# SxJyJay/MSMDFusion

Hardware: AMD Instinct MI355X
Metric: samples/sec MSMDFusion fwd+bwd nuScenes 0.075m voxel (MSMDFusion-LC sparse fusion path) (higher is better)
Workload: dtype f32 via 3xbf16 split MFMA (each fp32 operand = exact sum of 3 bf16 planes, 6 products, fp32 accumulate; fp32 storage); 1 GPU; configs[2]: MSMDFusion-LC sparse path (LiDAR SparseEncoder frozen + 4-scale virtual-point voxels + modality split + GMA-Conv + sparse_add + downscale -> BEV 640ch), fwd+bwd+AdamW, 2 x (28.7k LiDAR + 50k virtual pts)/GPU, 0.075 m voxels, fp32; global_batch=2, parallelism=dp1, index_prefetch=True, trainable_params=5654368

## Files before the change

### include/msmd_hip.h

```cpp
#ifndef MSMD_HIP_H_
#define MSMD_HIP_H_

#include <stddef.h>
#include <stdint.h>

#ifdef __cplusplus
extern "C" {
#endif

typedef void* msmd_stream_t;

enum msmd_status {
  MSMD_OK = 0,
  MSMD_ERR_INVALID_ARG = -1,
  MSMD_ERR_WORKSPACE = -2,
  MSMD_ERR_UNSUPPORTED = -3,
  MSMD_ERR_LAUNCH = -4,
  MSMD_ERR_RANGE = -5
};

const char* msmd_status_string(int status);
const char* msmd_last_launch_error(void);
int msmd_abi_version(void);
int msmd_device_ok(void);
// ... 122 lines not shown
  int32_t spatial_shape[3], ksize[3];
  int32_t method, reserved;
  int32_t* nbr;
} msmd_subm_desc;
size_t msmd_rulebook_subm3d_many_workspace_bytes(const msmd_subm_desc* descs, int n_desc);
int msmd_rulebook_subm3d_many(const msmd_subm_desc* descs, int n_desc, void* workspace,
                              size_t workspace_bytes, msmd_stream_t stream);

size_t msmd_rulebook_conv_workspace_bytes(int batch_size,
                                          const int* out_shape );

int msmd_rulebook_conv3d_count(const int32_t* indices , int n,
                               int batch_size, const int* out_shape,
                               const int* ksize, const int* stride,
                               const int* padding, int32_t* n_out ,
                               void* workspace, size_t workspace_bytes,
                               msmd_stream_t stream);

int msmd_rulebook_conv3d_fill(const int32_t* indices, int n, int batch_size,
                              const int* out_shape, const int* ksize,
                              const int* stride, const int* padding, int n_out,
                              int32_t* out_indices ,
                              int32_t* nbr_fwd ,
                              int32_t* nbr_bwd ,
                              void* workspace, size_t workspace_bytes,
                              msmd_stream_t stream);

int msmd_rulebook_deconv3d_count(const int32_t* indices , int n,
                                 int batch_size, const int* out_shape,
                                 const int* ksize, const int* stride,
                                 const int* padding, int32_t* n_out ,
                                 void* workspace, size_t workspace_bytes,
                                 msmd_stream_t stream);

int msmd_rulebook_deconv3d_fill(const int32_t* indices, int n, int batch_size,
                                const int* out_shape, const int* ksize,
                                const int* stride, const int* padding, int n_out,
                                int32_t* out_indices ,
                                int32_t* nbr_fwd ,
                                int32_t* nbr_bwd ,
                                void* workspace, size_t workspace_bytes,
                                msmd_stream_t stream);

size_t msmd_rulebook_conv_chain_workspace_bytes(int batch_size, int levels,
                                                const int* out_shapes);
int msmd_rulebook_conv3d_count_chain(const int32_t* indices, int n, int batch_size,
                                     int levels, const int* out_shapes, const int* ksizes,
                                     const int* strides, const int* paddings,
                                     int32_t* n_out , void* workspace,
                                     size_t workspace_bytes, msmd_stream_t stream);

size_t msmd_rulebook_add_conv_chain_workspace_bytes(int batch_size, int levels,
                                                    const int* in_shapes, const int* out_shapes);
int msmd_rulebook_add_conv_count_chain(const int32_t* const* extra, const int* n_extra,
                                       int batch_size, int levels, const int* in_shapes,
                                       const int* out_shapes, const int* ksizes,
                                       const int* strides, const int* paddings, int32_t* counts,
                                       void* workspace, size_t workspace_bytes,
                                       msmd_stream_t stream);

size_t msmd_rulebook_pairs_workspace_bytes(int kernel_volume, int n_rows);

int msmd_rulebook_pairs(const int32_t* nbr , int kernel_volume,
                        int n_rows, int32_t* indice_pairs ,
                        int ld, int32_t* indice_num , void* workspace,
                        size_t workspace_bytes, msmd_stream_t stream);

size_t msmd_spconv_packed_weight_elems(int kernel_volume, int c_in, int c_out);

int msmd_spconv_pack_weight(const float* weight, int kernel_volume, int c_in,
                            int c_out,
                            int flags ,
                            float* packed, msmd_stream_t stream);

int msmd_spconv_fwd_f32(const float* in_feat , int n_in,
                        int c_in, const float* packed_weight,
                        const int32_t* nbr , int ld, int n_out,
                        int kernel_volume, int weight_flip,
                        const int32_t* row_order ,
                        int32_t* tile_counter ,
                        float* out_feat , int c_out,
                        msmd_stream_t stream);

int msmd_spconv_fwd_split_supported(int c_in, int c_out, int kernel_volume);

size_t msmd_spconv_packed_split_bytes(int kernel_volume, int c_in ,
                                      int c_out , int planes);

int msmd_spconv_pack_weight_split(const float* weight, int kernel_volume, int c_in,
                                  int c_out, int flags ,
                                  int planes, void* packed, msmd_stream_t stream);
int msmd_spconv_pack_weight_split_pair(const float* weight, int kernel_volume, int c_in,
                                       int c_out, int flags, int planes, void* packed,
                                       void* packed_transposed, msmd_stream_t stream);

int msmd_spconv_pack_weight_split_many(const void* descs, int n_desc, long total_units,
                                       int planes, msmd_stream_t stream);

size_t msmd_spconv_fwd_split_workspace_bytes(int n_out, int c_out);

int msmd_spconv_fwd_split(const float* in_feat , int n_in, int c_in,
                          const void* packed_weight, const int32_t* nbr ,
                          int ld, int n_out, int kernel_volume, int weight_flip,
                          const int32_t* row_order ,
                          int32_t* tile_counter , int sync_ints,
                          float* out_feat , int c_out, int planes,
                          void* workspace, size_t workspace_bytes,
                          const int32_t* tile_prefix ,
                          msmd_stream_t stream);

int msmd_spconv_fwd_split_stats(const float* in_feat, int n_in, int c_in,
                                const void* packed_weight, const int32_t* nbr, int ld,
                                int n_out, int kernel_volume, int weight_flip,
                                const int32_t* row_order, int32_t* tile_counter, int sync_ints,
                                float* out_feat, int c_out, int planes, void* workspace,
                                size_t workspace_bytes, const int32_t* tile_prefix,
                                float* bn_partials, msmd_stream_t stream);
int msmd_spconv_fwd_split_stats_blocks(int n_out, int c_out);

int msmd_spconv_fwd_split_tile_rows(int c_out);

int msmd_spconv_fwd_split_instantiation(int c_out, int* params);

int msmd_rulebook_tile_prefix(const int32_t* nbr , int kernel_volume, int ld,
                              int n_rows, int rows_per_tile,
                              int32_t* prefix , msmd_stream_t stream);

int msmd_spconv_wgrad_split_supported(int c_in, int c_out);

int msmd_spconv_wgrad_split(const float* in_feat, int c_in, const float* d_out, int c_out,
                            const int32_t* indice_pairs ,
                            const int32_t* indice_num , int ld,
                            int kernel_volume, int planes,
                            float* d_weight ,
                            int krsc_out ,
                            void* workspace, size_t workspace_bytes, msmd_stream_t stream);

size_t msmd_rulebook_pair_segments_ints(int kernel_volume, int n_chunks);
int msmd_rulebook_pair_segments(const int32_t* indice_pairs ,
                                const int32_t* indice_num , int ld,
                                int kernel_volume, int chunk_rows, int n_chunks ,
                                int32_t* table ,
                                msmd_stream_t stream);
size_t msmd_spconv_wgrad_segments_workspace_bytes(int kernel_volume, int ld, int c_in, int c_out,
                                                  int n_chunks);
int msmd_spconv_wgrad_split_segments(const float* in_feat, int c_in, const float* d_out,
                                     int c_out, const int32_t* indice_pairs,
                                     const int32_t* indice_num, int ld, int kernel_volume,
                                     int planes, float* d_weight, int krsc_out,
                                     const int32_t* seg_table, int n_chunks, void* workspace,
                                     size_t workspace_bytes, msmd_stream_t stream);

int msmd_rulebook_permute_cols(const int32_t* nbr, int kernel_volume, int ld, int n,
                               const int32_t* order, int32_t* out ,
                               msmd_stream_t stream);

size_t msmd_rulebook_tiling_workspace_bytes(int n_rows, int rows_per_tile);
int msmd_rulebook_tiling(const int32_t* nbr, int kernel_volume, int n_rows,
                         int rows_per_tile, int32_t* order ,
                         int32_t* tiled , void* workspace,
                         size_t workspace_bytes, msmd_stream_t stream);

size_t msmd_rulebook_plan_workspace_bytes(int kernel_volume, int n_rows, int rows_per_tile);
int msmd_rulebook_plan(const int32_t* nbr, int kernel_volume, int n_rows,
                       int rows_per_tile, int32_t* order, int32_t* tiled,
                       int32_t* prefix128, int32_t* prefix256, int32_t* indice_pairs,
// ... 363 lines not shown
```

### msmdfusion_amd/_lib.py

```python
import ctypes as C
import os

import torch

_HERE = os.path.dirname(os.path.abspath(__file__))
LIB_PATH = os.environ.get("MSMD_LIB") or os.path.join(_HERE, "libmsmd_hip.so")

if not os.path.exists(LIB_PATH):
    raise RuntimeError(
        f"{LIB_PATH} is missing: the HIP library is not built. Run "
        "`make -C msmdfusion_amd/csrc` (hipcc, --offload-arch=gfx950). "
        "msmdfusion_amd has no fallback path.")

lib = (C.PyDLL if os.environ.get("MSMD_PYDLL") == "1" else C.CDLL)(LIB_PATH)

_vp, _i, _f, _sz = C.c_void_p, C.c_int, C.c_float, C.c_size_t
_i64 = C.c_int64
_ip = C.POINTER(C.c_int)
_fp = C.POINTER(C.c_float)

SIGNATURES = {
    "msmd_status_string": (C.c_char_p, [_i]),
    "msmd_last_launch_error": (C.c_char_p, []),
    "msmd_abi_version": (_i, []),
    "msmd_device_ok": (_i, []),
    "msmd_voxelize_workspace_bytes": (_sz, [_i, _i, _i]),
    "msmd_hard_voxelize": (_i, [_vp, _i, _i, _fp, _fp, _i, _i, _vp, _vp, _vp, _vp, _vp, _vp, _sz, _vp]),
    "msmd_hard_voxelize_many_workspace_bytes": (_sz, [_vp, _i]),
    "msmd_hard_voxelize_many": (_i, [_vp, _i, _vp, _sz, _vp]),
    "msmd_voxel_mean": (_i, [_vp, _vp, _i, _i, _i, _i, _vp, _vp]),
    "msmd_dynamic_voxelize": (_i, [_vp, _i, _i, _fp, _fp, _i, _vp, _vp]),
    "msmd_scatter_index_workspace_bytes": (_sz, [_i]),
    "msmd_scatter_index": (_i, [_vp, _i, _i, _vp, _vp, _vp, _vp, _vp, _vp, _vp, _sz, _vp]),
    "msmd_scatter_reduce_f32": (_i, [_vp, _i, _i, _vp, _vp, _i, _i, _vp, _vp, _vp]),
    "msmd_scatter_reduce_bwd_f32": (_i, [_vp, _i, _i, _i, _vp, _vp, _vp, _i, _vp, _vp]),
    "msmd_scatter_max_argmax_f32": (_i, [_vp, _i, _i, _vp, _vp, _i, _vp, _vp]),
    "msmd_scatter_gather_f32": (_i, [_vp, _i, _i, _vp, _i, _vp, _vp]),
    "msmd_roiaware_num_tiles": (_sz, [_i, _i]),
    "msmd_roiaware_count_workspace_bytes": (_sz, [_i, _i]),
    "msmd_roiaware_count": (_i, [_vp, _vp, _i, _vp, _vp, _i, _vp, _vp, _sz, _vp]),
    "msmd_roiaware_index_workspace_bytes": (_sz, [_i]),
    "msmd_roiaware_index": (_i, [_vp, _vp, _i, _vp, _vp, _i, _i, _i, _i, _i, _vp, _i, _vp, _vp, _vp,
                                 _vp, _vp, _sz, _vp]),
    "msmd_roiaware_pool_f32": (_i, [_vp, _i, _i, _vp, _vp, _i64, _i, _i, _i, _vp, _vp, _vp]),
    "msmd_roiaware_pool_bwd_f32": (_i, [_vp, _i64, _i, _vp, _i, _vp, _vp, _i, _vp, _i, _i, _vp, _vp]),
    "msmd_roiaware_write_table": (_i, [_vp, _vp, _i64, _i, _vp, _vp]),
    "msmd_roiaware_table_workspace_bytes": (_sz, [_i64, _i]),
    "msmd_roiaware_table_count": (_i, [_vp, _i64, _i, _vp, _vp, _sz, _vp]),
    "msmd_roiaware_table_index": (_i, [_vp, _i64, _i, _i, _i, _vp, _vp, _vp, _vp, _vp, _sz, _vp]),
    "msmd_points_in_boxes_f32": (_i, [_vp, _vp, _i, _i, _i, _i, _vp, _vp]),
    "msmd_rulebook_subm_workspace_bytes": (_sz, [_i]),
    "msmd_rulebook_subm3d": (_i, [_vp, _i, _i, _ip, _ip, _vp, _vp, _sz, _vp]),
    "msmd_rulebook_subm_bitmap_workspace_bytes": (_sz, [_i, _i, _ip]),
    "msmd_rulebook_subm3d_bitmap": (_i, [_vp, _i, _i, _ip, _ip, _vp, _vp, _sz, _vp]),
    "msmd_rulebook_conv_workspace_bytes": (_sz, [_i, _ip]),
    "msmd_rulebook_conv_chain_workspace_bytes": (_sz, [_i, _i, _ip]),
    "msmd_rulebook_conv3d_count_chain": (_i, [_vp, _i, _i, _i, _ip, _ip, _ip, _ip, _vp, _vp, _sz, _vp]),
    "msmd_rulebook_add_conv_chain_workspace_bytes": (_sz, [_i, _i, _ip, _ip]),
    "msmd_rulebook_add_conv_count_chain": (_i, [_vp, _ip, _i, _i, _ip, _ip, _ip, _ip, _ip, _vp, _vp,
                                                _sz, _vp]),
    "msmd_rulebook_conv3d_count": (_i, [_vp, _i, _i, _ip, _ip, _ip, _ip, _vp, _vp, _sz, _vp]),
    "msmd_rulebook_conv3d_fill": (_i, [_vp, _i, _i, _ip, _ip, _ip, _ip, _i, _vp, _vp, _vp, _vp, _sz, _vp]),
    "msmd_rulebook_deconv3d_count": (_i, [_vp, _i, _i, _ip, _ip, _ip, _ip, _vp, _vp, _sz, _vp]),
    "msmd_rulebook_deconv3d_fill": (_i, [_vp, _i, _i, _ip, _ip, _ip, _ip, _i, _vp, _vp, _vp, _vp, _sz,
                                         _vp]),
    "msmd_sparse_maxpool_fwd_f32": (_i, [_vp, _i, _i, _vp, _i, _i, _vp, _vp]),
    "msmd_sparse_maxpool_bwd_f32": (_i, [_vp, _vp, _vp, _i, _i, _vp, _i, _i, _vp, _vp]),
    "msmd_rulebook_pairs_workspace_bytes": (_sz, [_i, _i]),
    "msmd_rulebook_pairs": (_i, [_vp, _i, _i, _vp, _i, _vp, _vp, _sz, _vp]),
    "msmd_spconv_packed_weight_elems": (_sz, [_i, _i, _i]),
    "msmd_spconv_pack_weight": (_i, [_vp, _i, _i, _i, _i, _vp, _vp]),
    "msmd_spconv_fwd_f32": (_i, [_vp, _i, _i, _vp, _vp, _i, _i, _i, _i, _vp, _vp, _vp, _i, _vp]),
    "msmd_rulebook_row_masks": (_i, [_vp, _i, _i, _vp, _vp, _vp]),
    "msmd_rulebook_tile_costs": (_i, [_vp, _i, _i, _vp, _i, _vp, _vp]),
    "msmd_rulebook_tiling_workspace_bytes": (_sz, [_i, _i]),
    "msmd_rulebook_tiling": (_i, [_vp, _i, _i, _i, _vp, _vp, _vp, _sz, _vp]),
    "msmd_rulebook_plan_workspace_bytes": (_sz, [_i, _i, _i]),
    "msmd_rulebook_plan": (_i, [_vp, _i, _i, _i, _vp, _vp, _vp, _vp, _vp, _i, _vp, _vp, _sz, _vp]),
    "msmd_rulebook_subm3d_many_workspace_bytes": (_sz, [_vp, _i]),
    "msmd_rulebook_subm3d_many": (_i, [_vp, _i, _vp, _sz, _vp]),
    "msmd_rulebook_plan_many_workspace_bytes": (_sz, [_vp, _i]),
    "msmd_rulebook_plan_many": (_i, [_vp, _i, _vp, _sz, _vp]),
    "msmd_spconv_wgrad_workspace_bytes": (_sz, [_i, _i, _i, _i]),
    "msmd_spconv_wgrad_f32": (_i, [_vp, _i, _vp, _i, _vp, _vp, _i, _i, _vp, _i, _vp, _sz, _vp]),
    "msmd_spconv_packed_split_bytes": (_sz, [_i, _i, _i, _i]),
    "msmd_spconv_pack_weight_split": (_i, [_vp, _i, _i, _i, _i, _i, _vp, _vp]),
    "msmd_spconv_pack_weight_split_pair": (_i, [_vp, _i, _i, _i, _i, _i, _vp, _vp, _vp]),
    "msmd_spconv_fwd_split_supported": (_i, [_i, _i, _i]),
    "msmd_spconv_fwd_split_workspace_bytes": (_sz, [_i, _i]),
    "msmd_spconv_fwd_split": (_i, [_vp, _i, _i, _vp, _vp, _i, _i, _i, _i, _vp, _vp, _i, _vp, _i, _i,
                                   _vp, _sz, _vp, _vp]),
    "msmd_spconv_fwd_split_stats": (_i, [_vp, _i, _i, _vp, _vp, _i, _i, _i, _i, _vp, _vp, _i, _vp, _i, _i, _vp, _sz, _vp, _vp, _vp]),
    "msmd_rulebook_tile_prefix": (_i, [_vp, _i, _i, _i, _i, _vp, _vp]),
    "msmd_spconv_fwd_split_tile_rows": (_i, [_i]),
    "msmd_spconv_fwd_split_instantiation": (_i, [_i, _ip]),
    "msmd_spconv_fwd_split_stats_blocks": (_i, [_i, _i]),
    "msmd_spconv_wgrad_split_supported": (_i, [_i, _i]),
    "msmd_spconv_wgrad_split": (_i, [_vp, _i, _vp, _i, _vp, _vp, _i, _i, _i, _vp, _i, _vp, _sz, _vp]),
    "msmd_spconv_pack_weight_split_many": (_i, [_vp, _i, C.c_long, _i, _vp]),
    "msmd_rulebook_pair_segments_ints": (_sz, [_i, _i]),
    "msmd_rulebook_pair_segments": (_i, [_vp, _vp, _i, _i, _i, _i, _vp, _vp]),
    "msmd_spconv_wgrad_segments_workspace_bytes": (_sz, [_i, _i, _i, _i, _i]),
    "msmd_spconv_wgrad_split_segments": (_i, [_vp, _i, _vp, _i, _vp, _vp, _i, _i, _i, _vp, _i, _vp,
                                              _i, _vp, _sz, _vp]),
    "msmd_rulebook_permute_cols": (_i, [_vp, _i, _i, _i, _vp, _vp, _vp]),
    "msmd_bn_workspace_bytes": (_sz, [_i, _i]),
    "msmd_bn_act_fwd_f32": (_i, [_vp, _vp, _i, _i, _vp, _vp, _vp, _vp, _i, _f, _f, _i, _vp, _vp, _vp, _vp, _sz, _vp]),
    "msmd_bn_act_fwd_from_partials_f32": (_i, [_vp, _vp, _i, _i, _vp, _vp, _vp, _vp, _f, _f, _i, _vp,
                                               _vp, _vp, _vp, _i, _vp]),
    "msmd_bn_act_bwd_f32": (_i, [_vp, _vp, _vp, _i, _i, _vp, _vp, _vp, _i, _i, _vp, _vp, _vp, _vp, _vp, _sz, _vp]),
    "msmd_bn_relu_bwd_f32": (_i, [_vp, _vp, _i, _i, _vp, _vp, _vp, _vp, _i, _vp, _vp, _vp, _vp, _sz, _vp]),
    "msmd_dense_scatter_f32": (_i, [_vp, _vp, _i, _i, _i, _ip, _vp, _vp]),
    "msmd_dense_gather_f32": (_i, [_vp, _vp, _i, _i, _i, _ip, _vp, _vp]),
    "msmd_bev_scatter_nhwc_f32": (_i, [_vp, _vp, _i, _i, _i, _ip, _vp, _i, _i, _vp]),
    "msmd_bev_gather_nhwc_f32": (_i, [_vp, _vp, _i, _i, _i, _ip, _vp, _i, _i, _vp]),
    "msmd_fg_gather_f32": (_i, [_vp, _vp, _i, _i, _i, _i, _vp, _i, _vp, C.c_double, _vp, _i, _vp, _i,
                                _vp, _vp, _vp, _vp, _vp]),
    "msmd_fg_gather_scored_f32": (_i, [_vp, _vp, _i, _i, _i, _i, _vp, _i, _vp, C.c_double, _vp, _i, _vp,
                                       _vp, _vp, _i, _i, _vp, _vp, _vp]),
    "msmd_fg_scatter_add_f32": (_i, [_vp, _i, _i, _vp, _i, _i, _i, _i, _i, _vp, _vp, _vp]),
    "msmd_depth_canvas_workspace_bytes": (_sz, [_i, _i, _i]),
    "msmd_boxes_overlap_bev_f32": (_i, [_vp, _i, _vp, _i, _vp, _vp]),
    "msmd_boxes_iou3d_f32": (_i, [_vp, _i, _vp, _i, _vp, _i, _i, _i, _i, _vp, _vp]),
    "msmd_heatmap_gaussian_f32": (_i, [_vp, _vp, _vp, _vp, _i, _i, _i, _i, _vp, _vp]),
    "msmd_gaussian_focal_workspace_bytes": (_sz, [_i64]),
    "msmd_gaussian_focal_f32": (_i, [_vp, _vp, _i64, _f, _vp, _vp, _vp, _sz, _vp]),
    "msmd_boxes_iou_bev_f32": (_i, [_vp, _i, _vp, _i, _vp, _vp]),
    "msmd_nms_workspace_bytes": (_sz, [_i, _i]),
    "msmd_nms_batched_f32": (_i, [_i, _vp, _i, _vp, _i, _i, _i, _vp, _i, _vp, _vp, _i, _vp, _vp, _sz,
                                  _vp]),
    "msmd_depth_canvas_f32": (_i, [_vp, _i, _vp, _i, _i, _i, _i, _vp, _vp, _vp, _sz, _vp]),
    "msmd_sparse_add_workspace_bytes": (_sz, [_i, _ip]),
    "msmd_sparse_add_count": (_i, [_vp, _i, _vp, _i, _i, _ip, _vp, _vp, _sz, _vp]),
    "msmd_sparse_add_fill": (_i, [_vp, _vp, _i, _vp, _vp, _i, _i, _i, _ip, _i, _vp, _vp, _vp, _vp, _vp, _sz, _vp]),
    "msmd_sparse_add_rows": (_i, [_vp, _vp, _i, _vp, _vp, _i, _i, _i, _vp, _vp]),
    "msmd_rows_inverse": (_i, [_vp, _i, _i, _vp, _vp]),
    "msmd_sparse_add_rows_gather": (_i, [_vp, _vp, _vp, _i, _vp, _vp, _vp, _i, _i, _i, _vp, _vp]),
    "msmd_gma_assemble_fwd_f32": (_i, [_vp, _i, _i, _vp, _i, _i, _vp, _vp, _vp, _i, _i, _vp, _vp, _vp, _vp,
                                       _i, _i, _vp, _vp]),
    "msmd_gma_assemble_bwd_f32": (_i, [_vp, _i, _i, _i, _i, _vp, _vp, _vp, _i, _i, _vp, _i, _i, _vp, _vp,
                                       _vp, _vp, _vp, _vp, _vp]),
    "msmd_gma_assemble_bwd_workspace_floats": (_sz, [_i]),
    "msmd_rows_linear_supported": (_i, [_i, _i]),
    "msmd_rows_linear_fwd_f32": (_i, [_vp, _i, _vp, _i, _i, _vp, _vp, _i, _i, _vp, _vp]),
    "msmd_rows_linear_bwd_workspace_bytes": (_sz, [_i, _i, _i]),
    "msmd_rows_linear_bwd_f32": (_i, [_vp, _i, _vp, _i, _i, _vp, _vp, _i, _i, _vp, _vp, _vp, _sz,
                                      _vp]),
    "msmd_modality_split_workspace_bytes": (_sz, [_i, _ip]),
    "msmd_modality_split": (_i, [_vp, _i, _vp, _i, _i, _ip, _vp, _vp, _vp, _vp, _vp, _vp, _sz, _vp]),
    "msmd_modality_split_stats": (_i, [_vp, _i, _vp, _i, _i, _ip, _vp, _vp, _vp, _vp, _vp, _vp, _vp, _sz,
                                       _vp]),
    "msmd_modality_split_float_keys_workspace_bytes": (_sz, [_i, _i, _i]),
    "msmd_modality_split_float_keys": (_i, [_vp, _i, _vp, _i, _i, _ip, _vp, _vp, _vp, _vp, _vp, _vp, _i,
                                            _vp, _sz, _vp]),
    "msmd_rows_where_workspace_bytes": (_sz, [_i]),
# ... 64 lines not shown
```

### msmdfusion_amd/kernels.py

```python
import ctypes as C
import os

import torch

from ._lib import check, float_arr, int3, lib


def _raw_stream(device_index=None):
    if device_index is None:
        device_index = torch._C._cuda_getDevice()
    return torch._C._cuda_getCurrentRawStream(device_index)


def _stream():
    return C.c_void_p(_raw_stream())


def _p(t):
    return None if t is None else t.data_ptr()


def _need_cuda(*ts):
    cur = None
    for t in ts:
# ... 953 lines not shown
        if want_seg and (WGRAD_CHUNK_ROWS > 0 or ld <= 0):
            want_seg = False
        o = dict(kvol=kvol, n=n, ld=ld, order=take(n), tiled=take(kvol * n) if want_table else None,
                 prefix={r: take((n + r - 1) // r + 1) for r in sorted(rows)},
                 pairs=take(kvol * 2 * ld) if want_pairs else None,
                 num=take(kvol) if want_pairs else None,
                 seg=take(int(lib.msmd_rulebook_pair_segments_ints(kvol, 1))) if want_seg else None)
        lay.append(o)
        d.nbr, d.kvol, d.n_rows, d.ld = t.data_ptr(), kvol, n, ld
    slab = torch.empty((max(total, 1),), dtype=torch.int32, device=dev)
    base = slab.data_ptr()
    at = lambda off: None if off is None else base + 4 * off
    for d, o in zip(descs, lay):
        d.order, d.tiled = at(o["order"]), at(o["tiled"])
        d.prefix128, d.prefix256 = at(o["prefix"].get(128)), at(o["prefix"].get(256))
        d.indice_pairs, d.indice_num, d.segtab = at(o["pairs"]), at(o["num"]), at(o["seg"])
    nbytes = lib.msmd_rulebook_plan_many_workspace_bytes(descs, len(jobs))
    ws = _ws(nbytes, dev)
    check(lib.msmd_rulebook_plan_many(descs, len(jobs), _p(ws), nbytes, _stream()),
          "msmd_rulebook_plan_many")
    def view(off, *shape):
        size = 1
        for v in shape:
            size *= v
        return slab[off:off + size].view(*shape)
    out = []
    for o in lay:
        kvol, n, ld = o["kvol"], o["n"], o["ld"]
        pairs = None
        if o["pairs"] is not None:
            pairs = (view(o["pairs"], kvol, 2, ld), view(o["num"], kvol))
        seg = None
        if o["seg"] is not None:
            seg = (slab[o["seg"]:o["seg"] + 3 * kvol + 1], 1)
        out.append(dict(order=view(o["order"], n),
                        tiled=None if o["tiled"] is None else view(o["tiled"], kvol, n),
                        prefix={r: slab[off:off + (n + r - 1) // r + 1]
                                for r, off in o["prefix"].items()},
                        pairs=pairs, segments=seg))
    return out


_TILE_COUNTERS = {}


_SYNC_INTS = 1 + 8192


def _tile_counter(device):
    key = (device, _raw_stream(device.index))
    c = _TILE_COUNTERS.get(key)
    if c is None:
        c = _TILE_COUNTERS[key] = torch.zeros((_SYNC_INTS,), dtype=torch.int32, device=device)
    return c


_EXCHANGE = {}


def _exchange_buffer(device, nbytes):
    key = (device, _raw_stream(device.index))
    b = _EXCHANGE.get(key)
    if b is None or b.numel() < nbytes:
        b = _EXCHANGE[key] = torch.empty((max(int(nbytes), 256),), dtype=torch.uint8,
                                         device=device)
    return b


def conv_forward(feat, packed_weight, nbr, n_out, c_out, weight_flip=False, row_order=None):
    _need_cuda(feat, packed_weight, nbr)
    f = feat.contiguous().float()
    n_in, c_in = f.shape
    kvol, ld = nbr.shape
    out = torch.empty((n_out, c_out), dtype=torch.float32, device=f.device)
    counter = _tile_counter(f.device) if row_order is not None else None
    _launch("spconv_fwd", lambda: check(
        lib.msmd_spconv_fwd_f32(_p(f), n_in, c_in, _p(packed_weight), _p(nbr), ld, int(n_out),
                                kvol, int(bool(weight_flip)), _p(row_order), _p(counter),
                                _p(out), int(c_out), _stream()), "msmd_spconv_fwd_f32"),
            nbr=nbr, c_in=c_in, c_out=int(c_out), n_in=n_in, n_out=int(n_out))
    return out


_SPLIT_SUPPORTED = {}


def split_supported(c_in, c_out, kvol=27):
    key = (c_in, c_out, kvol)
    v = _SPLIT_SUPPORTED.get(key)
    if v is None:
        v = _SPLIT_SUPPORTED[key] = bool(
            lib.msmd_spconv_fwd_split_supported(int(c_in), int(c_out), int(kvol)))
    return v


def pack_weight_split(weight, planes=3, transpose=False, krsc=False):
    _need_cuda(weight)
    w = weight.contiguous().float()
    if krsc:
        cout, cin = w.shape[0], w.shape[-1]
        kvol = w.numel() // (cout * cin)
    else:
        kvol, cin, cout = w.shape
    ci, co = (cout, cin) if transpose else (cin, cout)
    packed = torch.empty((lib.msmd_spconv_packed_split_bytes(kvol, ci, co, planes),),
                         dtype=torch.uint8, device=w.device)
    check(lib.msmd_spconv_pack_weight_split(_p(w), kvol, cin, cout,
                                            int(bool(transpose)) | (2 if krsc else 0), planes,
                                            _p(packed), _stream()),
          "msmd_spconv_pack_weight_split")
    return packed


def pack_weight_split_pair(weight, planes=3, krsc=False):
    _need_cuda(weight)
    w = weight.contiguous().float()
    if krsc:
        cout, cin = w.shape[0], w.shape[-1]
        kvol = w.numel() // (cout * cin)
    else:
        kvol, cin, cout = w.shape
    a = torch.empty((lib.msmd_spconv_packed_split_bytes(kvol, cin, cout, planes),),
                    dtype=torch.uint8, device=w.device)
    b = torch.empty((lib.msmd_spconv_packed_split_bytes(kvol, cout, cin, planes),),
                    dtype=torch.uint8, device=w.device)
    check(lib.msmd_spconv_pack_weight_split_pair(_p(w), kvol, cin, cout, 2 if krsc else 0, planes,
                                                 _p(a), _p(b), _stream()),
          "msmd_spconv_pack_weight_split_pair")
    return a, b


class _PackDesc(C.Structure):
    _fields_ = [("w", C.c_void_p), ("packed_a", C.c_void_p), ("packed_b", C.c_void_p),
                ("start", C.c_int64), ("kvol", C.c_int32), ("cin", C.c_int32),
                ("cout", C.c_int32), ("flags", C.c_int32)]


def pack_weight_split_many(jobs, planes=3):
    if not jobs:
        return
    descs = (_PackDesc * len(jobs))()
    start = 0
    keep = []
    for i, (weight, krsc, packed, packed_t) in enumerate(jobs):
        _need_cuda(weight, packed, packed_t)
        w = weight.detach()
        if not (w.is_contiguous() and w.dtype == torch.float32):
            w = w.contiguous().float()
        keep.append(w)
        if krsc:
            cout, cin = w.shape[0], w.shape[-1]
            kvol = w.numel() // (cout * cin)
        else:
            kvol, cin, cout = w.shape
        d = descs[i]
        d.w, d.packed_a = w.data_ptr(), packed.data_ptr()
        d.packed_b = packed_t.data_ptr() if packed_t is not None else None
        d.start, d.kvol, d.cin, d.cout, d.flags = start, kvol, cin, cout, 2 if krsc else 0
        start += lib.msmd_spconv_packed_split_bytes(kvol, cin, cout, planes) // (16 * planes)
        if packed_t is not None:
            start += lib.msmd_spconv_packed_split_bytes(kvol, cout, cin, planes) // (16 * planes)
    dev = jobs[0][0].device
    host = torch.frombuffer(bytearray(bytes(descs)), dtype=torch.uint8).pin_memory()
    table = host.to(dev, non_blocking=True)
    check(lib.msmd_spconv_pack_weight_split_many(_p(table), len(jobs), start, int(planes),
                                                 _stream()), "msmd_spconv_pack_weight_split_many")
# ... 1212 lines not shown
```

### msmdfusion_amd/spconv/functional.py

```python
import os
from collections import namedtuple

import torch
from torch.autograd import Function

from .. import kernels as K


def conv_planes():
    return int(os.environ.get("MSMD_CONV_PLANES", "3"))


SPLIT_MAX_FEATURE_BYTES = 0xFFFFFF00


def _use_split(c_in, c_out, kvol, n_in=0, planes=None):
    return ((conv_planes() if planes is None else planes) in (1, 2, 3)
            and n_in * c_in * 4 < SPLIT_MAX_FEATURE_BYTES and K.split_supported(c_in, c_out, kvol))


ConvNeeds = namedtuple("ConvNeeds", "fwd bwd wgrad_split want_pairs want_segments planes")


def conv_needs(c_in, c_out, kvol, n_in, n_out, need_grad, is_subm):
    planes = conv_planes()

    def ask(side, ci, co, n):
        if _use_split(ci, co, kvol, n, planes):
            return side, "split", K.split_tile_rows(co)
        return side, "ordered" if co >= 64 and ci % 16 == 0 else "plain", None
    bwd = ask("fwd" if is_subm else "bwd", c_out, c_in, n_out) if need_grad else None
    wgs = bool(need_grad) and K.wgrad_split_supported(c_in, c_out)
    return ConvNeeds(ask("fwd", c_in, c_out, n_in), bwd, wgs and planes in (1, 2, 3),
                     bool(need_grad), wgs, planes)


_F32_TILE_COUNTS = (12, 8, 6, 5, 4, 3, 2, 1)


def _conv_f32(x, weight, krsc, transpose, nbr, n_out, weight_flip=False, row_order=None):
    if krsc:
        c_out = weight.shape[-1] if transpose else weight.shape[0]
    else:
        c_out = weight.shape[1] if transpose else weight.shape[2]
    tiles = (c_out + 15) // 16
    if tiles in _F32_TILE_COUNTS:
        return K.conv_forward(x, _pack_f32(weight, transpose, krsc), nbr,
                              n_out, c_out, weight_flip=weight_flip, row_order=row_order)
    outs, c0 = [], 0
    while c0 < c_out:
        left = (c_out - c0 + 15) // 16
        width = min(16 * next(t for t in _F32_TILE_COUNTS if t <= left), c_out - c0)
        if krsc:
            w = weight[..., c0:c0 + width] if transpose else weight[c0:c0 + width]
        else:
            w = weight[:, c0:c0 + width, :] if transpose else weight[:, :, c0:c0 + width]
        outs.append(K.conv_forward(x, K.pack_weight(w, transpose=transpose, krsc=krsc), nbr,
                                   n_out, width, weight_flip=weight_flip, row_order=row_order))
        c0 += width
    return torch.cat(outs, 1)


_PACKS = {}
_F32_PACKS = {}


def _pack_entry(weight, np_, krsc, want_t):
    import weakref
    wid = id(weight)
    key = (weight.data_ptr(), tuple(weight.shape), np_, krsc, weight.device)
    e = _PACKS.get(wid)
    if e is None or e["ref"]() is not weight or e["key"] != key:
        if krsc:
            cout, cin = weight.shape[0], weight.shape[-1]
            kvol = weight.numel() // (cout * cin)
        else:
            kvol, cin, cout = weight.shape
        e = dict(ref=weakref.ref(weight, lambda _r, wid=wid: _PACKS.pop(wid, None)), key=key,
                 dims=(kvol, cin, cout), version=None, packed_t=None,
                 packed=torch.empty((K.lib.msmd_spconv_packed_split_bytes(kvol, cin, cout, np_),),
                                    dtype=torch.uint8, device=weight.device))
        _PACKS[wid] = e
    if want_t and e["packed_t"] is None:
        kvol, cin, cout = e["dims"]
        e["packed_t"] = torch.empty((K.lib.msmd_spconv_packed_split_bytes(kvol, cout, cin, np_),),
                                    dtype=torch.uint8, device=weight.device)
        e["version"] = None
    return e


def _packed_parameter(weight, np_, krsc, want_t):
    e = _pack_entry(weight, np_, krsc, want_t)
    if e["version"] != weight._version:
        jobs, entries = [], []
        for o in list(_PACKS.values()):
            w = o["ref"]()
            if w is None or o["key"][2] != np_ or o["key"][4] != weight.device:
                continue
            if o["version"] != w._version:
                jobs.append((w, o["key"][3], o["packed"], o["packed_t"]))
                entries.append((o, w._version))
        K.pack_weight_split_many(jobs, np_)
        for o, v in entries:
            o["version"] = v
    return e["packed"], e["packed_t"]


def _pack_f32(weight, transpose, krsc):
    if not isinstance(weight, torch.nn.Parameter):
        return K.pack_weight(weight, transpose=transpose, krsc=krsc)
    import weakref
    ck = (id(weight), bool(transpose))
    key = (weight.data_ptr(), weight._version, krsc, tuple(weight.shape))
    hit = _F32_PACKS.get(ck)
    if hit is not None and hit[0]() is weight and hit[1] == key:
        return hit[2]
    packed = K.pack_weight(weight, transpose=transpose, krsc=krsc)
    _F32_PACKS[ck] = (weakref.ref(weight, lambda _r, ck=ck: _F32_PACKS.pop(ck, None)), key, packed)
    return packed


def invalidate_packed_weights(weight=None):
    if weight is None:
        for e in _PACKS.values():
            e["version"] = None
        _F32_PACKS.clear()
        return
    e = _PACKS.get(id(weight))
    if e is not None:
        e["version"] = None
    for t in (False, True):
        _F32_PACKS.pop((id(weight), t), None)


def _conv_forward(features, weight, rb, krsc, want_dgrad, bn_stats=False):
    c_in, c_out = (weight.shape[-1], weight.shape[0]) if krsc else weight.shape[1:]
    rb.check_ready()
    needs = conv_needs(c_in, c_out, rb.nbr_fwd.shape[0], features.shape[0], rb.n_out, want_dgrad,
                       rb.is_subm)
    _, kernel, rows = needs.fwd
    if kernel == "split":
        np_ = needs.planes
        packed_t = None
        want_t = want_dgrad and needs.bwd[1] == "split"
        if isinstance(weight, torch.nn.Parameter):
            packed, packed_t = _packed_parameter(weight, np_, krsc, want_t)
            packed_t = packed_t if want_t else None
        elif want_t:
            packed, packed_t = K.pack_weight_split_pair(weight, np_, krsc=krsc)
        else:
            packed = K.pack_weight_split(weight, np_, krsc=krsc)
        table, order = rb.fwd.tiling()
        res = K.conv_forward_split(features, packed, table, rb.n_out, c_out, np_,
                                   row_order=order, tile_prefix=rb.fwd.prefix(rows),
                                   bn_stats=bn_stats)
        return (res[0], packed_t, res[1]) if bn_stats else (res, packed_t)
    out = _conv_f32(features, weight, krsc, False, rb.nbr_fwd, rb.n_out,
                    row_order=rb.fwd.order() if kernel == "ordered" else None)
    return (out, None, None) if bn_stats else (out, None)


class _SparseConvFunction(Function):

    @staticmethod
    def forward(ctx, features, weight, rb, krsc, stats=None):
        ctx.rb, ctx.krsc = rb, krsc
        ctx.save_for_backward(features, weight)
        if stats is not None:
            out, ctx.packed_t, stats[0] = _conv_forward(features, weight, rb, krsc,
                                                        ctx.needs_input_grad[0], bn_stats=True)
        else:
            out, ctx.packed_t = _conv_forward(features, weight, rb, krsc, ctx.needs_input_grad[0])
        return out

    @staticmethod
    def backward(ctx, grad_out):
        features, weight = ctx.saved_tensors
        rb, krsc = ctx.rb, ctx.krsc
        c_in, c_out = (weight.shape[-1], weight.shape[0]) if krsc else weight.shape[1:]
        grad_out = grad_out.contiguous()
        d_feat = d_w = None
        needs = conv_needs(c_in, c_out, rb.nbr_fwd.shape[0], features.shape[0],
                           grad_out.shape[0], True, rb.is_subm)
        if ctx.needs_input_grad[1]:
            pairs, num = rb.pairs()
            if needs.wgrad_split:
                d_w = K.conv_wgrad_split(features, grad_out, pairs, num, needs.planes,
                                         krsc_shape=weight.shape if krsc else None,
                                         segments=rb.pair_segments())
            else:
                d_w = K.conv_wgrad(features, grad_out, pairs, num,
                                   krsc_shape=weight.shape if krsc else None)
        if ctx.needs_input_grad[0]:
            side, kernel, rows = needs.bwd
            side = getattr(rb, side)
            if kernel == "split":
                packed_t = ctx.packed_t if ctx.packed_t is not None else \
                    K.pack_weight_split(weight, needs.planes, transpose=True, krsc=krsc)
                table, order = side.tiling()
                d_feat = K.conv_forward_split(grad_out, packed_t, table, rb.n_in, c_in,
                                              needs.planes, weight_flip=rb.is_subm,
                                              row_order=order, tile_prefix=side.prefix(rows))
            else:
                d_feat = _conv_f32(grad_out, weight, krsc, True, side.nbr, rb.n_in,
                                   weight_flip=rb.is_subm,
                                   row_order=side.order() if kernel == "ordered" else None)
        return d_feat, d_w, None, None, None


def sparse_conv(features, weight, rb, krsc=False, bn_stats=None):
    if not (torch.is_grad_enabled() and (features.requires_grad or weight.requires_grad)):
        if bn_stats is not None:
            out, _, bn_stats[0] = _conv_forward(features, weight, rb, krsc, False, bn_stats=True)
            return out
        return _conv_forward(features, weight, rb, krsc, False)[0]
    return _SparseConvFunction.apply(features, weight, rb, krsc, bn_stats)


class _BNActFunction(Function):

    @staticmethod
    def forward(ctx, x, residual, gamma, beta, running_mean, running_var, training, momentum,
                eps, relu, stats=None):
        y, mean, invstd = K.bn_act_forward(x, residual, gamma, beta, running_mean, running_var,
                                           training, momentum, eps, relu, partials=stats)
        ctx.save_for_backward(x, y, gamma, beta, mean, invstd)
        ctx.cfg = (bool(training), bool(relu), residual is not None)
        return y

    @staticmethod
    def backward(ctx, dy):
        x, y, gamma, beta, mean, invstd = ctx.saved_tensors
        training, relu, has_res = ctx.cfg
        if relu and not has_res and gamma.dtype == torch.float32 and beta.dtype == torch.float32:
            dx, dgamma, dbeta = K.bn_relu_backward(x, dy, gamma, beta, mean, invstd, training)
            return dx, None, dgamma, dbeta, None, None, None, None, None, None, None
        dx, dres, dgamma, dbeta = K.bn_act_backward(x, y, dy, gamma, mean, invstd, training, relu,
                                                    has_res and ctx.needs_input_grad[1])
# ... 197 lines not shown
```

Before: 170.9 samples/s.

## Add narrow-channel sparse conv forward kernel with fp32 MFMA and fused BN stats

```diff
diff --git a/include/msmd_hip.h b/include/msmd_hip.h
--- a/include/msmd_hip.h
+++ b/include/msmd_hip.h
@@ -228,6 +228,14 @@
                         float* out_feat , int c_out,
                         msmd_stream_t stream);
 
+int msmd_spconv_fwd_narrow_supported(int c_in, int c_out, int kernel_volume);
+int msmd_spconv_fwd_narrow_stats_blocks(int n_out, int c_out);
+int msmd_spconv_fwd_narrow(const float* in_feat , int n_in, int c_in,
+                           const float* packed_weight, const int32_t* nbr ,
+                           int ld, int n_out, int kernel_volume, int weight_flip,
+                           float* out_feat , int c_out,
+                           float* bn_partials , msmd_stream_t stream);
+
 int msmd_spconv_fwd_split_supported(int c_in, int c_out, int kernel_volume);
 
 size_t msmd_spconv_packed_split_bytes(int kernel_volume, int c_in ,
diff --git a/msmdfusion_amd/_lib.py b/msmdfusion_amd/_lib.py
--- a/msmdfusion_amd/_lib.py
+++ b/msmdfusion_amd/_lib.py
@@ -71,6 +71,9 @@
     "msmd_spconv_packed_weight_elems": (_sz, [_i, _i, _i]),
     "msmd_spconv_pack_weight": (_i, [_vp, _i, _i, _i, _i, _vp, _vp]),
     "msmd_spconv_fwd_f32": (_i, [_vp, _i, _i, _vp, _vp, _i, _i, _i, _i, _vp, _vp, _vp, _i, _vp]),
+    "msmd_spconv_fwd_narrow_supported": (_i, [_i, _i, _i]),
+    "msmd_spconv_fwd_narrow_stats_blocks": (_i, [_i, _i]),
+    "msmd_spconv_fwd_narrow": (_i, [_vp, _i, _i, _vp, _vp, _i, _i, _i, _i, _vp, _i, _vp, _vp]),
     "msmd_rulebook_row_masks": (_i, [_vp, _i, _i, _vp, _vp, _vp]),
     "msmd_rulebook_tile_costs": (_i, [_vp, _i, _i, _vp, _i, _vp, _vp]),
     "msmd_rulebook_tiling_workspace_bytes": (_sz, [_i, _i]),
diff --git a/msmdfusion_amd/csrc/spconv_narrow.hip b/msmdfusion_amd/csrc/spconv_narrow.hip
--- /dev/null
+++ b/msmdfusion_amd/csrc/spconv_narrow.hip
@@ -0,0 +1,225 @@
+#include "common.hpp"
+
+namespace msmd {
+namespace {
+
+typedef float f32x4 __attribute__((ext_vector_type(4)));
+
+constexpr int kNarrowRows = 128;
+constexpr int kNarrowSteps = 28;
+
+template <int NT, int T, int R, int WV, bool VEC>
+__global__ __launch_bounds__(WV * 64) void spconv_fwd_narrow_kernel(
+    const float* __restrict__ in, int cin, const float* __restrict__ wp,
+    const int32_t* __restrict__ nbr, int ld, int n_out, int kvol, int flip,
+    float* __restrict__ out, int cout, float* __restrict__ bn_part) {
+  static_assert(R * WV * 16 == kNarrowRows, "one tile is 128 rows");
+  extern __shared__ __attribute__((aligned(16))) char smem[];
+  f32x4* wl = (f32x4*)smem;
+  float* stat = (float*)(wl + kvol * T * NT * 64);
+  const int tid = threadIdx.x, lane = tid & 63;
+  const int wave = __builtin_amdgcn_readfirstlane(tid >> 6);
+  const int j = lane & 15, q = lane >> 4;
+  const int n_tiles = (n_out + kNarrowRows - 1) / kNarrowRows;
+
+  for (int e = tid; e < kvol * T * NT * 64; e += WV * 64) wl[e] = ((const f32x4*)wp)[e];
+  __syncthreads();
+
+  for (int tile = blockIdx.x; tile < n_tiles; tile += gridDim.x) {
+    int rows[R];
+    int nbq[R][7];
+#pragma unroll
+    for (int r = 0; r < R; ++r) {
+      const int p = tile * kNarrowRows + (wave * R + r) * 16 + j;
+      rows[r] = p < n_out ? p : -1;
+#pragma unroll
+      for (int i = 0; i < 7; ++i) {
+        const int k = 4 * i + q;
+        nbq[r][i] = (rows[r] >= 0 && k < kvol) ? nbr[(size_t)k * ld + rows[r]] : -1;
+      }
+    }
+    f32x4 acc[R][NT];
+#pragma unroll
+    for (int r = 0; r < R; ++r)
+#pragma unroll
+      for (int n = 0; n < NT; ++n) acc[r][n] = (f32x4){0.f, 0.f, 0.f, 0.f};
+
+    f32x4 b[3][R][T];
+    bool any[3];
+    auto gather = [&](int k, f32x4 (&bk)[R][T], bool& anyk) {
+      bool a = false;
+#pragma unroll
+      for (int r = 0; r < R; ++r) {
+        const int src = __shfl(nbq[r][k >> 2], ((k & 3) << 4) | j, 64);
+        a |= src >= 0;
+#pragma unroll
+        for (int t = 0; t < T; ++t) {
+          f32x4 v = (f32x4){0.f, 0.f, 0.f, 0.f};
+          const int c0 = 16 * t + 4 * q;
+          if (src >= 0) {
+            const float* p = in + (size_t)src * cin + c0;
+            if (VEC) {
+              if (c0 < cin) v = *(const f32x4*)p;
+            } else {
+#pragma unroll
+              for (int s = 0; s < 4; ++s)
+                if (c0 + s < cin) v[s] = p[s];
+            }
+          }
+          bk[r][t] = v;
+        }
+      }
+      anyk = __any(a);
+    };
+    gather(0, b[0], any[0]);
+    gather(1, b[1], any[1]);
+#pragma unroll
+    for (int k = 0; k < kNarrowSteps; ++k) {
+      if (k + 2 < kNarrowSteps) gather(k + 2, b[(k + 2) % 3], any[(k + 2) % 3]);
+      if (!any[k % 3]) continue;
+      const f32x4* wk = wl + (size_t)(flip ? kvol - 1 - k : k) * (T * NT * 64) + lane;
+#pragma unroll
+      for (int t = 0; t < T; ++t) {
+        if (R >= 2) {
+#pragma unroll
+          for (int n = 0; n < NT; ++n) {
+            const f32x4 a = wk[(t * NT + n) * 64];
+#pragma unroll
+            for (int s = 0; s < 4; ++s)
+#pragma unroll
+              for (int r = 0; r < R; ++r)
+                acc[r][n] = __builtin_amdgcn_mfma_f32_16x16x4f32(a[s], b[k % 3][r][t][s],
+                                                                 acc[r][n], 0, 0, 0);
+          }
+        } else {
+          f32x4 a[NT];
+#pragma unroll
+          for (int n = 0; n < NT; ++n) a[n] = wk[(t * NT + n) * 64];
+#pragma unroll
+          for (int s = 0; s < 4; ++s)
+#pragma unroll
+            for (int n = 0; n < NT; ++n)
+              acc[0][n] = __builtin_amdgcn_mfma_f32_16x16x4f32(a[n][s], b[k % 3][0][t][s],
+                                                               acc[0][n], 0, 0, 0);
+        }
+      }
+    }
+
+#pragma unroll
+    for (int r = 0; r < R; ++r) {
+      if (rows[r] < 0) continue;
+      float* o = out + (size_t)rows[r] * cout;
+#pragma unroll
+      for (int n = 0; n < NT; ++n) {
+        const int c0 = 16 * n + 4 * q;
+        if ((cout & 3) == 0) {
+          if (c0 < cout) *(f32x4*)(o + c0) = acc[r][n];
+        } else {
+#pragma unroll
+          for (int s = 0; s < 4; ++s)
+            if (c0 + s < cout) o[c0 + s] = acc[r][n][s];
+        }
+      }
+    }
+
+    if (bn_part) {
+      float* st_w = stat + wave * (2 * NT * 16);
+#pragma unroll
+      for (int n = 0; n < NT; ++n) {
+        f32x4 s1 = {0.f, 0.f, 0.f, 0.f}, s2 = {0.f, 0.f, 0.f, 0.f};
+#pragma unroll
+        for (int r = 0; r < R; ++r) {
+          s1 += acc[r][n];
+          s2 += acc[r][n] * acc[r][n];
+        }
+#pragma unroll
+        for (int m = 1; m < 16; m <<= 1)
+#pragma unroll
+          for (int e = 0; e < 4; ++e) {
+            s1[e] += __shfl_xor(s1[e], m, 64);
+            s2[e] += __shfl_xor(s2[e], m, 64);
+          }
+        if (j == 0) {
+          *(f32x4*)(st_w + 16 * n + 4 * q) = s1;
+          *(f32x4*)(st_w + NT * 16 + 16 * n + 4 * q) = s2;
+        }
+      }
+      __syncthreads();
+      if (tid < 2 * NT * 16) {
+        float v = 0.f;
+#pragma unroll
+        for (int w2 = 0; w2 < WV; ++w2) v += stat[w2 * (2 * NT * 16) + tid];
+        const int which = tid >= NT * 16 ? 1 : 0, c = tid - which * NT * 16;
+        if (c < cout) bn_part[((size_t)tile * 2 + which) * cout + c] = v;
+      }
+      __syncthreads();
+    }
+  }
+}
+
+template <int NT, int T, int R, int WV, bool VEC>
+int launch_narrow(const float* in, int cin, const float* wp, const int32_t* nbr, int ld,
+                  int n_out, int kvol, int flip, float* out, int cout, float* bn_part,
+                  hipStream_t st) {
+  const size_t image = sizeof(f32x4) * (size_t)kvol * T * NT * 64;
+  const size_t smem = image + sizeof(float) * WV * 2 * NT * 16;
+  int per_cu = (int)((160 * 1024) / smem);
+  if (per_cu > 32 / WV) per_cu = 32 / WV;
+  int nblk = ceil_div(n_out, kNarrowRows);
+  if (nblk > 256 * per_cu) nblk = 256 * per_cu;
+  auto kern = spconv_fwd_narrow_kernel<NT, T, R, WV, VEC>;
+  static LdsGrant granted;
+  const int lds_rc = optin_dynamic_lds((const void*)kern, smem, granted);
+  if (lds_rc != MSMD_OK) return lds_rc;
+  MSMD_LAUNCH(kern, dim3(nblk), dim3(WV * 64), smem, st, in, cin, wp, nbr, ld, n_out, kvol, flip,
+              out, cout, bn_part);
+  return launch_status();
+}
+
+}
+}
+using namespace msmd;
+
+MSMD_EXPORT int msmd_spconv_fwd_narrow_supported(int c_in, int c_out, int kernel_volume) {
+  return c_in >= 1 && c_in <= 32 && c_out >= 1 && c_out <= 32 && kernel_volume >= 1 &&
+         kernel_volume <= kNarrowSteps;
+}
+
+MSMD_EXPORT int msmd_spconv_fwd_narrow_stats_blocks(int n_out, int c_out) {
+  (void)c_out;
+  return ceil_div(n_out > 0 ? n_out : 0, kNarrowRows);
+}
+
+MSMD_EXPORT int msmd_spconv_fwd_narrow(const float* in_feat, int n_in, int c_in,
+                                       const float* packed_weight, const int32_t* nbr, int ld,
+                                       int n_out, int kernel_volume, int weight_flip,
+                                       float* out_feat, int c_out, float* bn_partials,
+                                       msmd_stream_t stream) {
+  if (n_in < 0 || n_out < 0 || c_in < 1 || c_out < 1 || kernel_volume < 1 || ld < n_out)
+    return MSMD_ERR_INVALID_ARG;
+  if (!msmd_spconv_fwd_narrow_supported(c_in, c_out, kernel_volume)) return MSMD_ERR_UNSUPPORTED;
+  if (n_out == 0) return MSMD_OK;
+  if (!packed_weight || !nbr || !out_feat || (n_in > 0 && !in_feat)) return MSMD_ERR_INVALID_ARG;
+  hipStream_t st = (hipStream_t)stream;
+  const int T = (c_in + 15) / 16, NT = (c_out + 15) / 16;
+  const bool vec = (c_in & 3) == 0;
+#define NARROW(NTv, Tv, Rv, WVv, VECv)                                                       \
+  return launch_narrow<NTv, Tv, Rv, WVv, VECv>(in_feat, c_in, packed_weight, nbr, ld, n_out, \
+                                               kernel_volume, weight_flip, out_feat, c_out,  \
+                                               bn_partials, st)
+  if (T == 1 && NT == 1) {
+    if (vec) NARROW(1, 1, 2, 4, true);
+    NARROW(1, 1, 2, 4, false);
+  }
+  if (T == 1 && NT == 2) {
+    if (vec) NARROW(2, 1, 2, 4, true);
+    NARROW(2, 1, 2, 4, false);
+  }
+  if (T == 2 && NT == 1) {
+    if (vec) NARROW(1, 2, 2, 4, true);
+    NARROW(1, 2, 2, 4, false);
+  }
+  if (vec) NARROW(2, 2, 1, 8, true);
+  NARROW(2, 2, 1, 8, false);
+#undef NARROW
+}
diff --git a/msmdfusion_amd/kernels.py b/msmdfusion_amd/kernels.py
--- a/msmdfusion_amd/kernels.py
+++ b/msmdfusion_amd/kernels.py
@@ -1059,6 +1059,32 @@
     return out
 
 
+def narrow_supported(c_in, c_out, kvol=27):
+    return bool(lib.msmd_spconv_fwd_narrow_supported(int(c_in), int(c_out), int(kvol)))
+
+
+def conv_forward_narrow(feat, packed_weight, nbr, n_out, c_out, weight_flip=False,
+                        bn_stats=False):
+    _need_cuda(feat, packed_weight, nbr)
+    f = feat.contiguous().float()
+    n_in, c_in = f.shape
+    kvol, ld = nbr.shape
+    out = torch.empty((n_out, c_out), dtype=torch.float32, device=f.device)
+    part = None
+    if int(n_out) > 0:
+        if bn_stats:
+            part = torch.empty((int(lib.msmd_spconv_fwd_narrow_stats_blocks(int(n_out),
+                                                                            int(c_out))), 2,
+                                int(c_out)), dtype=torch.float32, device=f.device)
+        _launch("spconv_fwd", lambda: check(
+            lib.msmd_spconv_fwd_narrow(_p(f), n_in, c_in, _p(packed_weight), _p(nbr), ld,
+                                       int(n_out), kvol, int(bool(weight_flip)), _p(out),
+                                       int(c_out), _p(part), _stream()),
+            "msmd_spconv_fwd_narrow"),
+                nbr=nbr, c_in=c_in, c_out=int(c_out), n_in=n_in, n_out=int(n_out))
+    return (out, part) if bn_stats else out
+
+
 _SPLIT_SUPPORTED = {}
 
 
diff --git a/msmdfusion_amd/spconv/functional.py b/msmdfusion_amd/spconv/functional.py
--- a/msmdfusion_amd/spconv/functional.py
+++ b/msmdfusion_amd/spconv/functional.py
@@ -25,14 +25,21 @@
 def conv_needs(c_in, c_out, kvol, n_in, n_out, need_grad, is_subm):
     planes = conv_planes()
 
-    def ask(side, ci, co, n):
+    def ask(side, ci, co, n, forward=False):
+        if forward and ci % 4 == 0 and K.narrow_supported(ci, co, kvol):
+            return side, "narrow", None
         if _use_split(ci, co, kvol, n, planes):
             return side, "split", K.split_tile_rows(co)
         return side, "ordered" if co >= 64 and ci % 16 == 0 else "plain", None
     bwd = ask("fwd" if is_subm else "bwd", c_out, c_in, n_out) if need_grad else None
     wgs = bool(need_grad) and K.wgrad_split_supported(c_in, c_out)
-    return ConvNeeds(ask("fwd", c_in, c_out, n_in), bwd, wgs and planes in (1, 2, 3),
+    return ConvNeeds(ask("fwd", c_in, c_out, n_in, True), bwd, wgs and planes in (1, 2, 3),
                      bool(need_grad), wgs, planes)
+
+
+def _narrow_forward(kernel, c_in, c_out, kvol):
+    return kernel == "narrow" or (kernel == "plain" and c_in % 4 != 0
+                                  and K.narrow_supported(c_in, c_out, kvol))
 
 
 _F32_TILE_COUNTS = (12, 8, 6, 5, 4, 3, 2, 1)
@@ -154,6 +161,13 @@
         res = K.conv_forward_split(features, packed, table, rb.n_out, c_out, np_,
                                    row_order=order, tile_prefix=rb.fwd.prefix(rows),
                                    bn_stats=bn_stats)
+        return (res[0], packed_t, res[1]) if bn_stats else (res, packed_t)
+    if _narrow_forward(kernel, c_in, c_out, rb.nbr_fwd.shape[0]):
+        res = K.conv_forward_narrow(features, _pack_f32(weight, False, krsc), rb.nbr_fwd, rb.n_out,
+                                    c_out, bn_stats=bn_stats)
+        packed_t = None
+        if want_dgrad and needs.bwd[1] == "split" and isinstance(weight, torch.nn.Parameter):
+            packed_t = _packed_parameter(weight, needs.planes, krsc, True)[1]
         return (res[0], packed_t, res[1]) if bn_stats else (res, packed_t)
     out = _conv_f32(features, weight, krsc, False, rb.nbr_fwd, rb.n_out,
                     row_order=rb.fwd.order() if kernel == "ordered" else None)
```

Result: no change. 171.0 samples/s (median of 3 runs) (+0.1%).
